# 0xPolygonZero/proof-protocol-decoder

Hardware: AMD Instinct MI355X
Metric: txn-proofs/sec (whole node), 256-txn synthetic block (higher is better)
Workload: dtype u64 (Goldilocks field)

## Files before the change

### include/bpg.h

```cpp
#ifndef BPG_H
#define BPG_H
#include <stddef.h>
#include <stdint.h>

#ifdef __cplusplus
extern "C" {
#endif

typedef enum {
  BP_OK = 0,
  BP_ERR_ABORTED = -1,
  BP_ERR_INVALID_INPUT = -2,
  BP_ERR_RANGE = -3,
  BP_ERR_DEVICE = -4,
  BP_ERR_VERIFY = -5,
  BP_ERR_UNSUPPORTED = -6
} bp_status;

const char* bp_last_error(void);
const char* bp_version(void);
int bp_device_count(void);
int bp_use_blocking_sync(int device);
int bp_host_wait_mode(int device);



#define BP_NTT_MAX_COLS 65535u

enum { BP_NTT_FWD_BR2NAT = 0, BP_NTT_INV_NAT2BR = 1, BP_NTT_FWD_NAT = 2, BP_NTT_INV_NAT = 3 };
int bp_ntt_batch(uint64_t* d_cols, uint32_t log_n, uint32_t n_cols, uint64_t col_stride, int dir,
                 void* stream);

int bp_intt_batch(const uint64_t* d_values, uint64_t in_stride, uint64_t* d_coeffs_out, uint64_t out_stride,
                  uint32_t log_n, uint32_t n_cols, void* stream);

int bp_lde_batch(const uint64_t* d_in, uint64_t in_stride, uint64_t* d_coeffs_out, uint64_t coeffs_stride,
                 uint64_t* d_lde_out, uint64_t lde_stride, uint32_t log_n, uint32_t rate_bits,
                 uint32_t n_cols, int from_coeffs, void* stream);

int bp_debug_copy_u64(const uint64_t* d_in, uint64_t* d_out, uint64_t n, void* stream);

int bp_debug_field_ops(const uint64_t* d_a, const uint64_t* d_b, uint64_t* d_out, uint64_t n, void* stream);
int bp_debug_mul_pow2(const uint64_t* d_a, uint64_t* d_out, uint64_t n, void* stream);

void bp_tune_quad_threshold(uint64_t n_perms);
void bp_tune_merkle_fused(int mode);
void bp_tune_merkle_wide(int log2_parents);
void bp_tune_poseidon_mx(int on);
void bp_tune_poseidon_mx_sets(int sets);
void bp_tune_poseidon_grouped(int on);
void bp_tune_assume_loaded(int mode);
void bp_tune_rec_batch(int n);
void bp_tune_side_lanes(int n);
void bp_tune_rec_riders(int on);
void bp_tune_txn_group(int n);
void bp_tune_rec_group(int mode);
int bp_debug_rec_batch_histogram(uint64_t* out, uint32_t n, int reset);
void bp_tune_witness_threads(int n);
void bp_tune_host_wait(int mode);
void bp_tune_host_poseidon(int mode);
int bp_debug_poseidon_host(uint64_t* states, size_t n);
void bp_tune_k5_spread(int on);
uint32_t bp_debug_poseidon_group_ops(uint32_t K);
int bp_debug_poseidon_group_tables(uint32_t K, uint32_t r0, uint8_t* out_ops, int32_t* out_cform, int32_t* out_cmain,
                                   int32_t* out_max_plane_sum);
// ... 326 lines not shown
```

### proof_protocol_decoder_amd/_abi.py

```python
import ctypes as C
from ctypes import POINTER as P

vp, cp, i, sz, dbl = C.c_void_p, C.c_char_p, C.c_int, C.c_size_t, C.c_double
u8, u32, u64, i32, i64 = C.c_uint8, C.c_uint32, C.c_uint64, C.c_int32, C.c_int64
u8p, u32p, u64p, i32p, szp = P(u8), P(u32), P(u64), P(i32), P(sz)
u8pp = P(u8p)

BP_OK, BP_ERR_ABORTED, BP_ERR_INVALID_INPUT, BP_ERR_RANGE, BP_ERR_DEVICE, BP_ERR_VERIFY, BP_ERR_UNSUPPORTED = 0, -1, -2, -3, -4, -5, -6
STATUS_NAMES = {v: k for k, v in list(globals().items()) if k == "BP_OK" or k.startswith("BP_ERR_")}
BP_SET_SKIP_LINK_CHECK = 1
BP_NUM_TABLES, BP_IR_WORDS, BP_PV_WORDS = 7, 25, 13

KNOBS = ("quad_threshold", "assume_loaded", "merkle_fused", "merkle_wide", "poseidon_mx", "poseidon_mx_sets",
         "poseidon_grouped", "ntt_mx", "ntt_split", "k5_spread", "host_wait", "host_poseidon", "rec_batch",
         "witness_threads", "side_lanes")


def _u32s(*names):
    return [(n, u32) for n in names]


class AirFamily(C.Structure):
    _fields_ = _u32s("first_index", "count", "kind", "degree")

# ... 96 lines not shown

class ShardOptions(C.Structure):
    _fields_ = _u32s("n_threads", "tree_shape")


ShardLeafFn = C.CFUNCTYPE(i, vp, u32, u8pp, szp)
ShardAggFn = C.CFUNCTYPE(i, vp, u8p, sz, i, u8p, sz, i, u8pp, szp)

_cfg, _conf, _wit, _opt, _gi = P(StarkCfg), P(BpConfig), P(TxnWitness), P(ShardOptions), P(GiOptions)
_trace = (i, [vp, u64, u32, vp, vp])
_check = [u32, _cfg, vp, u64, vp, u64p, u32, u64p, u32p, P(AirViolation), u32, u32p]
_knob, _ir_flag, _buf = (None, [i]), (i, [u64p, i]), [u8pp, szp]
PROTOTYPES = {
    "bp_last_error": (cp, []),
    "bp_version": (cp, []),
    "bp_device_count": (i, []),
    "bp_use_blocking_sync": (i, [i]),
    "bp_host_wait_mode": (i, [i]),
    "bp_ntt_batch": (i, [vp, u32, u32, u64, i, vp]),
    "bp_intt_batch": (i, [vp, u64, vp, u64, u32, u32, vp]),
    "bp_lde_batch": (i, [vp, u64, vp, u64, vp, u64, u32, u32, u32, i, vp]),
    "bp_debug_copy_u64": (i, [vp, vp, u64, vp]),
    "bp_debug_field_ops": (i, [vp, vp, vp, u64, vp]),
    "bp_debug_mul_pow2": (i, [vp, vp, u64, vp]),
    "bp_tune_quad_threshold": (None, [u64]),
    "bp_tune_merkle_fused": _knob,
    "bp_tune_merkle_wide": _knob,
    "bp_tune_poseidon_mx": _knob,
    "bp_tune_poseidon_mx_sets": _knob,
    "bp_tune_poseidon_grouped": _knob,
    "bp_tune_assume_loaded": _knob,
    "bp_tune_rec_batch": _knob,
    "bp_tune_side_lanes": _knob,
    "bp_tune_rec_riders": _knob,
    "bp_tune_txn_group": _knob,
    "bp_tune_rec_group": _knob,
    "bp_debug_rec_batch_histogram": (i, [u64p, u32, i]),
    "bp_tune_witness_threads": _knob,
    "bp_tune_host_wait": _knob,
    "bp_tune_host_poseidon": _knob,
    "bp_debug_poseidon_host": (i, [vp, sz]),
    "bp_tune_k5_spread": _knob,
    "bp_debug_poseidon_group_ops": (u32, [u32]),
    "bp_debug_poseidon_group_tables": (i, [u32, u32, u8p, i32p, i32p, i32p]),
    "bp_tune_ntt_split": _knob,
    "bp_tune_ntt_mx": _knob,
# ... 103 lines not shown
```

### proof_protocol_decoder_amd/csrc/air.hpp

```cpp
#pragma once
#include <cstdint>
#include <type_traits>
#include "gl.hpp"
#if defined(__HIP__)
#include "poseidon.cuh"
#endif

namespace bpg {
namespace air {

constexpr uint32_t SYNTHETIC = 0, KECCAK_F = 1, LOGIC = 2, MEMORY = 3, ARITHMETIC = 4, BYTE_PACKING = 5, KECCAK_SPONGE = 6, ARITHMETIC_MUL = 7, PLONK = 8, COUNT = 9;

struct Shape {
  uint32_t air_id, n_cols, n_const, deg_pow;
};

template <class T>
struct Ops;

#if defined(__HIP__)
template <>
struct Ops<uint64_t> {
  typedef uint64_t T;
  static __device__ __forceinline__ T k(uint64_t c) { return c; }
  static __device__ __forceinline__ T add(T a, T b) { return gl::addc(a, b); }
  static __device__ __forceinline__ T sub(T a, T b) { return gl::subc(a, b); }
  static __device__ __forceinline__ T mul(T a, T b) { return gl::mulc(a, b); }
  static __device__ __forceinline__ T dbl(T a) { return gl::addc(a, a); }
  static __device__ __forceinline__ void mul4(const T (&a)[4], const T (&b)[4], T (&r)[4]) {
    __builtin_amdgcn_sched_barrier(0);
    gl::mul_n<4>(a, b, r);
    gl::canon_n<4>(r);
    __builtin_amdgcn_sched_barrier(0);
  }
  static __device__ __forceinline__ void mul4_lazy(const T (&a)[4], const T (&b)[4], T (&r)[4]) {
    __builtin_amdgcn_sched_barrier(0);
    gl::mul_n<4>(a, b, r);
    __builtin_amdgcn_sched_barrier(0);
  }
  static __device__ __forceinline__ T add_lazy(T a_any, T b) { return gl::add(a_any, b); }
  static __device__ __forceinline__ T sub_lazy(T a_any, T b) { return gl::sub(a_any, b); }
  static __device__ __forceinline__ T mul7(T a_any) { return gl::mul7(a_any); }
};
#endif
template <>
struct Ops<gl::Ext> {
  typedef gl::Ext T;
  static T k(uint64_t c) { return gl::ext(c); }
  static T add(T a, T b) { return gl::add(a, b); }
  static T sub(T a, T b) { return gl::sub(a, b); }
  static T mul(T a, T b) { return gl::mul(a, b); }
  static T dbl(T a) { return gl::add(a, a); }
  static void mul4(const T (&a)[4], const T (&b)[4], T (&r)[4]) {
    for (int i = 0; i < 4; i++) r[i] = gl::mul(a[i], b[i]);
  }
  static void mul4_lazy(const T (&a)[4], const T (&b)[4], T (&r)[4]) { mul4(a, b, r); }
  static T add_lazy(T a, T b) { return gl::add(a, b); }
  static T sub_lazy(T a, T b) { return gl::sub(a, b); }
  static T mul7(T a) { return gl::scale(a, 7); }
};

GL_HD uint64_t poseidon_rc(uint32_t i) {
  constexpr uint64_t RC[360] = {
#include "poseidon_rc.inc"
  };
  return RC[i];
}
GL_HD uint32_t poseidon_mds_entry(uint32_t r, uint32_t c) {
  constexpr uint32_t C[12] = {17, 15, 41, 16, 2, 28, 13, 13, 39, 18, 34, 20};
  return C[(c + 12 - r) % 12] + ((r | c) == 0 ? 8u : 0u);
}
template <class T>
struct PoseidonOps {
  typedef Ops<T> F;
  static GL_HD T sbox(T x) {
    const T x2 = F::mul(x, x), x4 = F::mul(x2, x2), x3 = F::mul(x2, x);
    return F::mul(x3, x4);
  }
  static GL_HD void sbox_all(T (&s)[12]) {
    for (uint32_t i = 0; i < 12; i++) s[i] = sbox(s[i]);
  }
  static GL_HD void mds_rc(T (&s)[12], int next) {
    T o[12];
    for (uint32_t r = 0; r < 12; r++) {
      T acc = F::k(next >= 0 ? poseidon_rc(12 * (uint32_t)next + r) : 0);
      for (uint32_t c = 0; c < 12; c++) acc = F::add(acc, F::mul(F::k(poseidon_mds_entry(r, c)), s[c]));
      o[r] = acc;
    }
    for (uint32_t r = 0; r < 12; r++) s[r] = o[r];
  }
  static GL_HD void mds_rc_word0(T (&s)[12], int next) { mds_rc(s, next); }
  static GL_HD T add_rc0(T x, uint32_t i) { return F::add(x, F::k(poseidon_rc(i))); }
};
#if defined(__HIP__)
template <>
struct PoseidonOps<uint64_t> {
  static __device__ __forceinline__ uint64_t sbox(uint64_t x) { return gl::canon(poseidon::sbox(x)); }
  static __device__ __forceinline__ void sbox_all(uint64_t (&s)[12]) { poseidon::sbox_all(s); }
  static __device__ __forceinline__ void mds_rc(uint64_t (&s)[12], int next) {
    if (next >= 0) poseidon::mds<true>(s, poseidon::RC + 12 * next);
    else poseidon::mds<false>(s, nullptr);
#pragma unroll
    for (int i = 0; i < 12; i++) s[i] = gl::canon(s[i]);
  }
  static __device__ __forceinline__ void mds_rc_word0(uint64_t (&s)[12], int next) {
    poseidon::mds<true>(s, poseidon::RC + 12 * next);
    s[0] = gl::canon(s[0]);
  }
  static __device__ __forceinline__ uint64_t add_rc0(uint64_t x, uint32_t i) { return gl::addc(x, poseidon::RC[i]); }
};
#endif

namespace synthetic {
GL_HD uint32_t n_constraints(const Shape& s) { return 3 * (s.n_cols / 4); }
GL_HD uint32_t per_unit(const Shape& s) {
  const uint32_t G = s.n_cols / 4, u = (G + 47) / 48;
  return u < 8 ? 8 : u;
}
GL_HD uint32_t n_units(const Shape& s) {
  const uint32_t G = s.n_cols / 4, pu = per_unit(s);
  return (G + pu - 1) / pu;
}
template <class T, class Row, class Emit>
GL_HD void eval_unit(const Shape& s, uint32_t unit, const Row& row, Emit& out) {
  typedef Ops<T> F;
  const uint32_t G = s.n_cols / 4, pu = per_unit(s), g0 = unit * pu, g1 = g0 + pu < G ? g0 + pu : G;
#pragma unroll 1
  for (uint32_t g = g0; g < g1; g++) {
    const T a = row.loc(4 * g), b = row.loc(4 * g + 1), c = row.loc(4 * g + 2), d = row.loc(4 * g + 3);
    const T dn = row.nxt(4 * g + 3);
    const T q = s.n_const ? row.cst(g % s.n_const) : F::k(1);
    const T x4[4] = {a, q, a, a}, y4[4] = {b, a, b, b};
    T p4[4];
    F::mul4(x4, y4, p4);
    const T ab = p4[0], qa = p4[1];
    T t = F::mul(ab, c);
    if (s.deg_pow == 3) t = F::mul(F::mul(t, t), t);
    out.all(3 * g, F::sub(F::sub(c, ab), qa));
    out.transition(3 * g + 1, F::sub(F::sub(dn, t), b));
    out.first(3 * g + 2, F::sub(F::sub(d, a), b));
  }
}
}

namespace keccak {
constexpr uint32_t N_COLS = 2431, N_CONSTRAINTS = 2826, N_UNITS = 11;
constexpr uint32_t COL_STEP = 0, COL_A = 24, COL_C = 74, COL_CP = 394, COL_AP = 714, COL_APP = 2314, COL_APP0_BITS = 2364,
                   COL_APPP = 2428, COL_G = 2430;
constexpr uint32_t F0 = 0, F1 = 24, F2 = 48, F3 = 2032, F4 = 2352, F5 = 2672, F6 = 2722, F7 = 2772, F8 = 2774, F9 = 2776;
GL_HD uint64_t round_constant(uint32_t i) {
  constexpr uint64_t RC[24] = {
      0x0000000000000001ULL, 0x0000000000008082ULL, 0x800000000000808aULL, 0x8000000080008000ULL,
      0x000000000000808bULL, 0x0000000080000001ULL, 0x8000000080008081ULL, 0x8000000000008009ULL,
      0x000000000000008aULL, 0x0000000000000088ULL, 0x0000000080008009ULL, 0x000000008000000aULL,
      0x000000008000808bULL, 0x800000000000008bULL, 0x8000000000008089ULL, 0x8000000000008003ULL,
      0x8000000000008002ULL, 0x8000000000000080ULL, 0x000000000000800aULL, 0x800000008000000aULL,
      0x8000000080008081ULL, 0x8000000000008080ULL, 0x0000000080000001ULL, 0x8000000080008008ULL};
  return RC[i];
}
GL_HD uint32_t rho(uint32_t l) {
  constexpr uint8_t R[25] = {0, 1, 62, 28, 27, 36, 44, 6, 55, 20, 3, 10, 43, 25, 39, 41, 45, 15, 21, 8, 18, 2, 61, 56, 14};
  return R[l];
}
// ... 665 lines not shown
#pragma unroll
    for (uint32_t i = 0; i < 4; i++) {
      lhs[i] = row.loc(H_IN + i);
      rhs[i] = row.loc(H_IN + 4 + i);
      dl[i] = row.loc(H_DELTA + i);
      pr[i] = F::sub(rhs[i], lhs[i]);
    }
    const T s4[4] = {sw, sw, sw, sw};
    F::mul4(s4, pr, g);
#pragma unroll
    for (uint32_t i = 0; i < 4; i++) {
      const T d = F::sub(dl[i], g[i]);
      out.all(G5 + 1 + i, SELECTOR ? F::mul(qh, d) : d);
      st[i] = H::add_rc0(F::add(lhs[i], dl[i]), i);
      st[4 + i] = H::add_rc0(F::sub(rhs[i], dl[i]), 4 + i);
      st[8 + i] = H::add_rc0(row.loc(H_IN + 8 + i), 8 + i);
    }
    const T bit = F::mul(sw, F::sub(sw, F::k(1)));
    out.all(G5, SELECTOR ? F::mul(qh, bit) : bit);
  }
  auto check12 = [&](uint32_t col0, uint32_t idx0) {
#pragma unroll
    for (uint32_t i0 = 0; i0 < 12; i0 += 4) {
      T d[4], g[4];
#pragma unroll
      for (uint32_t i = 0; i < 4; i++) {
        const T wv = row.loc(col0 + i0 + i);
        d[i] = F::sub(wv, st[i0 + i]);
        st[i0 + i] = wv;
      }
      if (SELECTOR) F::mul4(q4, d, g);
#pragma unroll
      for (uint32_t i = 0; i < 4; i++) out.all(idx0 + i0 + i, SELECTOR ? g[i] : d[i]);
    }
  };
#pragma unroll 1
  for (uint32_t r = 1; r <= 3; r++) {
    H::sbox_all(st);
    H::mds_rc(st, (int)r);
    check12(H_FULL1 + 12 * (r - 1), G4 + 12 * (r - 1));
  }
  H::sbox_all(st);
  H::mds_rc_word0(st, 4);
#pragma unroll 1
  for (uint32_t r = 4; r <= 25; r++) {
    const T pv = row.loc(H_PART + r - 4);
    const T d = F::sub(pv, st[0]);
    out.all(G4 + 36 + (r - 4), SELECTOR ? F::mul(qh, d) : d);
    st[0] = H::sbox(pv);
    if (r < 25) H::mds_rc_word0(st, (int)r + 1);
    else H::mds_rc(st, (int)r + 1);
  }
#pragma unroll 1
// ... 3 lines not shown
    H::mds_rc(st, r < 29 ? (int)r + 1 : -1);
  }
  check12(H_OUT, G4 + 106);
}
template <class T, class Row, class Emit>
GL_HD void eval_chunk_unit(uint32_t u, uint32_t ctl_base, const uint64_t ctl[4], const Row& row, Emit& out) {
  typedef Ops<T> F;
  T w[8], sg[8];
#pragma unroll
  for (uint32_t i = 0; i < 8; i++) w[i] = row.loc(8 * u + i);
#pragma unroll
  for (uint32_t i = 0; i < 8; i++) sg[i] = row.cst(CST_SIGMA + 8 * u + i);
  const T qa = row.cst(CST_ARITH), qs = row.cst(CST_SBOX), c0 = row.cst(CST_C0), c1 = row.cst(CST_C1);
  const T x = row.x(), kp = F::k(chunk_shift(u));
  const T beta[2] = {F::k(ctl[0]), F::k(ctl[2])}, gamma[2] = {F::k(ctl[1]), F::k(ctl[3])};
  T bkx[2];
  {
    const T l1[4] = {w[0], w[4], c1, c1}, r1[4] = {w[1], w[5], w[2], w[6]};
    T p1[4];
    F::mul4(l1, r1, p1);
    const T l2[4] = {c0, c0, beta[0], beta[1]}, r2[4] = {p1[0], p1[1], x, x};
    T p2[4];
    F::mul4(l2, r2, p2);
    const T t0 = F::sub(F::add(p2[0], p1[2]), w[3]), t1 = F::sub(F::add(p2[1], p1[3]), w[7]);
    const T l3[4] = {qa, qa, p2[2], p2[3]}, r3[4] = {t0, t1, kp, kp};
    T p3[4];
    F::mul4(l3, r3, p3);
    out.all(G0 + 2 * u, p3[0]);
    out.all(G0 + 2 * u + 1, p3[1]);
    bkx[0] = p3[2];
    bkx[1] = p3[3];
  }
  T half[2][4];
#pragma unroll
  for (uint32_t c = 0; c < 2; c++) {
    const T b4[4] = {beta[c], beta[c], beta[c], beta[c]};
    T pn[4], pd[4];
#pragma unroll
    for (uint32_t h = 0; h < 2; h++) {
      const T s4[4] = {sg[4 * h], sg[4 * h + 1], sg[4 * h + 2], sg[4 * h + 3]};
      T bs[4], tn[4], td[4];
      F::mul4_lazy(b4, s4, bs);
#pragma unroll
      for (uint32_t i = 0; i < 4; i++) {
        const T wg = F::add(w[4 * h + i], gamma[c]);
        tn[i] = F::add_lazy(bkx[c], wg);
        td[i] = F::add_lazy(bs[i], wg);
        bkx[c] = F::mul7(bkx[c]);
      }
      const T l4[4] = {tn[0], tn[2], td[0], td[2]}, r4[4] = {tn[1], tn[3], td[1], td[3]};
      T q4[4];
      F::mul4_lazy(l4, r4, q4);
      pn[2 * h] = q4[0]; pn[2 * h + 1] = q4[1]; pd[2 * h] = q4[2]; pd[2 * h + 1] = q4[3];
    }
    const T l4[4] = {pn[0], pn[2], pd[0], pd[2]}, r4[4] = {pn[1], pn[3], pd[1], pd[3]};
    F::mul4_lazy(l4, r4, half[c]);
  }
  {
    const T l4[4] = {half[0][0], half[0][2], half[1][0], half[1][2]}, r4[4] = {half[0][1], half[0][3], half[1][1], half[1][3]};
    T nd[4];
    F::mul4_lazy(l4, r4, nd);
    const uint32_t k = u + 1;
    T cur[2], prev[2];
#pragma unroll
    for (uint32_t c = 0; c < 2; c++) {
      cur[c] = row.aux(10 * c + (k < 10 ? k : 0));
      prev[c] = k == 1 ? row.aux_nxt(10 * c) : row.aux(10 * c + k - 1);
    }
    const T m4[4] = {cur[0], prev[0], cur[1], prev[1]}, n4[4] = {nd[1], nd[0], nd[3], nd[2]};
    T g4[4];
    F::mul4(m4, n4, g4);
    out.all(ctl_base + u, F::sub(g4[0], g4[1]));
    out.all(ctl_base + 11 + u, F::sub(g4[2], g4[3]));
    if (u == 9) {
      out.first(ctl_base + 10, F::sub(cur[0], F::k(1)));
      out.first(ctl_base + 21, F::sub(cur[1], F::k(1)));
    }
  }
  if (u < 6) {
    const uint32_t n_here = u < 5 ? 2 : 1;
    const T qs4[4] = {qs, qs, qs, qs};
    T pend[4] = {F::k(0), F::k(0), F::k(0), F::k(0)};
#pragma unroll
    for (uint32_t e = 0; e < 2; e++) {
      if (e >= n_here) break;
      const uint32_t i = 2 * u + e, col = COL_SBOX + 5 * i;
      const T xs = row.loc(col), x2 = row.loc(col + 1), x4 = row.loc(col + 2), x6 = row.loc(col + 3), x7 = row.loc(col + 4);
      const T l4[4] = {xs, x2, x4, x6}, r4[4] = {xs, x2, x2, xs};
      T p4[4], d4[4], g4[4];
      F::mul4(l4, r4, p4);
      d4[0] = F::sub(x2, p4[0]); d4[1] = F::sub(x4, p4[1]); d4[2] = F::sub(x6, p4[2]); d4[3] = F::sub(x7, p4[3]);
      F::mul4(qs4, d4, g4);
#pragma unroll
      for (uint32_t q = 0; q < 4; q++) out.all(G1 + 4 * i + q, g4[q]);
      pend[2 * e] = F::sub(xs, w[4 * e]);
      pend[2 * e + 1] = F::sub(x7, w[4 * e + 3]);
    }
    T w4[4];
    F::mul4(qs4, pend, w4);
    out.all(G2 + 4 * u, w4[0]);
    out.all(G2 + 4 * u + 1, w4[1]);
    if (n_here == 2) {
      out.all(G2 + 4 * u + 2, w4[2]);
      out.all(G2 + 4 * u + 3, w4[3]);
    }
  }
  if (u == 0) {
#pragma unroll
    for (uint32_t j = 0; j < 4; j++) out.first(G3 + j, F::sub(w[j], F::k(row.pub(j))));
  }
}
template <class T, class Row, class Emit>
GL_HD void eval_unit(uint32_t u, uint32_t ctl_base, const uint64_t ctl[4], const Row& row, Emit& out) {
  if (u == 10) eval_hash_unit<T>(row, out);
// ... 306 lines not shown
```

### proof_protocol_decoder_amd/csrc/gl.hpp

```cpp
#pragma once
#include <cstdint>
#include <hip/hip_runtime.h>

#define GL_HD __host__ __device__ __forceinline__

namespace gl {

constexpr uint64_t P = 0xFFFFFFFF00000001ULL;
constexpr uint64_t EPS = 0xFFFFFFFFULL;
constexpr uint64_t GENERATOR = 7;
constexpr uint64_t TWO_ADIC_ROOT = 1753635133440165772ULL;
constexpr uint64_t W = 7;

#if defined(__HIP__)
namespace cc {
typedef uint64_t mask;
__device__ __forceinline__ uint64_t mad_co(uint32_t a, uint32_t b, uint64_t c, mask& co) {
  uint64_t d;
  asm("v_mad_u64_u32 %0, %1, %2, %3, %4" : "=v"(d), "=s"(co) : "v"(a), "v"(b), "v"(c));
  return d;
}
__device__ __forceinline__ uint64_t mad_eps_co(uint32_t a, uint64_t c, mask& co) {
  uint64_t d;
  asm("v_mad_u64_u32 %0, %1, %2, -1, %3" : "=v"(d), "=s"(co) : "v"(a), "v"(c));
// ... 20 lines not shown
  return d;
}
__device__ __forceinline__ uint32_t sub_co(uint32_t a, uint32_t b, mask& co) {
  uint32_t d;
  asm("v_sub_co_u32_e64 %0, %1, %2, %3" : "=v"(d), "=s"(co) : "v"(a), "v"(b));
  return d;
}
__device__ __forceinline__ uint32_t subb_co(uint32_t a, uint32_t b, mask ci, mask& co) {
  uint32_t d;
  asm("s_nop 1\n\tv_subb_co_u32_e64 %0, %1, %2, %3, %4" : "=v"(d), "=s"(co) : "v"(a), "v"(b), "s"(ci));
  return d;
}
__device__ __forceinline__ uint32_t subb0_co(uint32_t a, mask ci, mask& co) {
  uint32_t d;
  asm("s_nop 1\n\tv_subbrev_co_u32_e64 %0, %1, 0, %2, %3" : "=v"(d), "=s"(co) : "v"(a), "s"(ci));
  return d;
}
__device__ __forceinline__ uint32_t sel_eps(mask m) {
  uint32_t d;
  asm("s_nop 1\n\tv_cndmask_b32_e64 %0, 0, -1, %1" : "=v"(d) : "s"(m));
  return d;
}
__device__ __forceinline__ uint64_t mk64(uint32_t lo, uint32_t hi) { return ((uint64_t)hi << 32) | lo; }
#include "gl_cc.inc"
}
#endif
GL_HD uint64_t canon(uint64_t a) {
  return a >= P ? a - P : a;
}

GL_HD uint64_t add(uint64_t a, uint64_t b) {
  uint64_t s = a + b;
  return s < b ? s + EPS : s;
}
GL_HD uint64_t sub(uint64_t a, uint64_t b) {
  uint64_t d = a - b;
  return a < b ? d - EPS : d;
}
GL_HD uint64_t addc(uint64_t a, uint64_t b) {
  uint64_t s = a + b;
  return (s < a || s >= P) ? s - P : s;
}
GL_HD uint64_t subc(uint64_t a, uint64_t b) {
  return a >= b ? a - b : a + (P - b);
}
GL_HD uint64_t negc(uint64_t a) {
  return a ? P - a : 0;
}

GL_HD uint64_t reduce128(uint64_t lo, uint64_t hi) {
  uint64_t hh = hi >> 32, hl = hi & EPS;
  uint64_t t0 = lo - hh;
  if (lo < hh) t0 -= EPS;
  uint64_t t1 = (hl << 32) - hl;
  uint64_t r = t0 + t1;
  return r < t1 ? r + EPS : r;
}

GL_HD void mul_wide(uint64_t a, uint64_t b, uint64_t& lo, uint64_t& hi) {
#if defined(__HIP_DEVICE_COMPILE__)
  uint32_t a0 = (uint32_t)a, a1 = (uint32_t)(a >> 32), b0 = (uint32_t)b, b1 = (uint32_t)(b >> 32);
  uint64_t p00 = (uint64_t)a0 * b0;
  uint64_t mid = (uint64_t)a0 * b1 + (p00 >> 32);
  uint64_t mid2 = (uint64_t)a1 * b0 + (uint32_t)mid;
  hi = (uint64_t)a1 * b1 + (mid >> 32) + (mid2 >> 32);
  lo = (mid2 << 32) | (uint32_t)p00;
#else
  unsigned __int128 x = (unsigned __int128)a * b;
  lo = (uint64_t)x;
  hi = (uint64_t)(x >> 64);
// ... 98 lines not shown
  cc::subb_co_o(hi, b2, ah, bh, b1);
  cc::addc0_co(lo, b3, b2);
#pragma unroll
  for (int i = 0; i < N; i++) b2[i] &= ~b3[i];
  cc::subb0_cv(hi, b2);
#pragma unroll
  for (int i = 0; i < N; i++) r[i] = cc::mk64(lo[i], hi[i]);
}
template <int N>
__device__ __forceinline__ void canon_n(uint64_t (&a)[N]) {
  uint32_t lo[N], hi[N], tl[N], th[N];
  cc::mask k[N], c[N];
#pragma unroll
  for (int i = 0; i < N; i++) {
    lo[i] = (uint32_t)a[i]; hi[i] = (uint32_t)(a[i] >> 32);
  }
  cc::add_m1_co_o(tl, k, lo);
  cc::addc0_co_o(th, c, hi, k);
  cc::sel(lo, tl, c);
  cc::sel(hi, th, c);
#pragma unroll
  for (int i = 0; i < N; i++) a[i] = cc::mk64(lo[i], hi[i]);
}
#endif
GL_HD uint64_t mul_pow2_portable(uint64_t x, unsigned S) {
  if (S < 64) return reduce128(x << S, S ? x >> (64 - S) : 0);
  const unsigned s = S - 64;
  const uint64_t lo = x << s, hi = s ? x >> (64 - s) : 0;
  return sub(reduce128(0, lo), hi << 32);
}
#if defined(__HIP__)
__device__ __forceinline__ void shl96(uint64_t x, int s, uint32_t& l0, uint32_t& l1, uint32_t& l2) {
  const uint32_t x0 = (uint32_t)x, x1 = (uint32_t)(x >> 32);
  l0 = x0 << s;
  l1 = (x1 << s) | (x0 >> (32 - s));
  l2 = x1 >> (32 - s);
}
__device__ __forceinline__ uint64_t mul_pow2_lo(uint64_t x, int s) {
  uint32_t l0, l1, l2;
  shl96(x, s, l0, l1, l2);
  cc::mask c3, b3, cx;
  const uint64_t V = cc::mad_eps_co(l2, cc::mk64(l0, l1), c3);
  const uint32_t t0 = cc::subb0_co((uint32_t)V, c3, b3);
  const uint32_t t1 = cc::addc0_co((uint32_t)(V >> 32), c3 & ~b3, cx);
  return cc::mk64(t0, t1);
}
// ... 166 lines not shown
  const uint64_t e30 = mul(sq_n(e24, 6), e6);
  const uint64_t e31 = mul(sq_n(e30, 1), e1);
  const uint64_t hi = sq_n(e31, 1);
  const uint64_t lo = mul(hi, a);
  return mulc(sq_n(hi, 32), lo);
}
GL_HD uint64_t root(unsigned k) {
  uint64_t r = TWO_ADIC_ROOT;
  for (unsigned i = k; i < 32; i++) r = mulc(r, r);
  return r;
}

struct Ext {
  uint64_t c0, c1;
};
GL_HD Ext ext(uint64_t a, uint64_t b = 0) { return Ext{a, b}; }
GL_HD bool eq(Ext a, Ext b) { return a.c0 == b.c0 && a.c1 == b.c1; }
GL_HD Ext add(Ext a, Ext b) { return Ext{addc(a.c0, b.c0), addc(a.c1, b.c1)}; }
GL_HD Ext sub(Ext a, Ext b) { return Ext{subc(a.c0, b.c0), subc(a.c1, b.c1)}; }
GL_HD uint64_t mul7(uint64_t x) {
  const uint64_t p = (uint64_t)(uint32_t)x * 7u;
  const uint64_t m = (x >> 32) * 7u + (p >> 32);
  const uint64_t u = (m << 32) | (uint32_t)p;
  const uint64_t t = u + (m >> 32) * EPS;
  return t < u ? t + EPS : t;
}
GL_HD Ext mul(Ext a, Ext b) {
#if defined(__HIP_DEVICE_COMPILE__)
  const uint64_t x[4] = {a.c0, a.c1, a.c0, a.c1}, y[4] = {b.c0, b.c1, b.c1, b.c0};
  uint64_t r[4];
  mul_n<4>(x, y, r);
  return Ext{addc(canon(r[0]), canon(mul7(r[1]))), addc(canon(r[2]), canon(r[3]))};
#else
  uint64_t c0 = addc(mulc(a.c0, b.c0), mulc(W, mulc(a.c1, b.c1)));
  uint64_t c1 = addc(mulc(a.c0, b.c1), mulc(a.c1, b.c0));
  return Ext{c0, c1};
#endif
}
GL_HD Ext scale(Ext a, uint64_t s) { return Ext{mulc(a.c0, s), mulc(a.c1, s)}; }
GL_HD Ext pow(Ext a, uint64_t e) {
  Ext r = ext(1);
  while (e) {
    if (e & 1) r = mul(r, a);
    a = mul(a, a);
    e >>= 1;
  }
  return r;
}
GL_HD Ext inv(Ext a) {
  uint64_t n = subc(mulc(a.c0, a.c0), mulc(W, mulc(a.c1, a.c1)));
  uint64_t ni = inv(n);
  return Ext{mulc(a.c0, ni), mulc(negc(a.c1), ni)};
}

GL_HD uint32_t bitrev(uint32_t x, unsigned bits) {
// ... 11 lines not shown
```

### proof_protocol_decoder_amd/csrc/hash_kernels.hip

```cpp
#include <atomic>
#include <cstring>
#include <memory>
#include <mutex>
#include <vector>
#include "common.hpp"
#include "poseidon.cuh"
#include "poseidon_mx.cuh"
#include "stark_kernels.hpp"
#include "tune.hpp"

namespace {

__global__ void __launch_bounds__(256) perm_batch_kernel(uint64_t* __restrict__ states, uint64_t n) {
  uint64_t i = blockIdx.x * (uint64_t)blockDim.x + threadIdx.x;
  if (i >= n) return;
  uint64_t s[12];
#pragma unroll
  for (int k = 0; k < 12; k++) s[k] = states[i * 12 + k];
  poseidon::permute(s);
#pragma unroll
  for (int k = 0; k < 12; k++) states[i * 12 + k] = gl::canon(s[k]);
}

__global__ void __launch_bounds__(256) __attribute__((amdgpu_waves_per_eu(4, 8)))
// ... 482 lines not shown
    if (i >= n) break;
    const uint64_t cb = gl::canon(y[k]);
    out[0 * n + i] = gl::canon(gl::mul(x[k], y[k]));
    out[1 * n + i] = gl::canon(r4[k]);
    out[2 * n + i] = k ? gl::canon(r3[k - 1]) : gl::canon(r4[0]);
    uint64_t lo, hi;
    gl::mul_wide(x[k], y[k], lo, hi);
    out[3 * n + i] = gl::canon(gl::reduce128(lo, hi));
    out[4 * n + i] = gl::canon(gl::add(x[k], cb));
    out[5 * n + i] = gl::canon(gl::sub(x[k], cb));
    out[6 * n + i] = gl::dot_reduce(d[k]);
    out[7 * n + i] = gl::canon(gl::mul7(x[k]));
    out[8 * n + i] = gl::inv(gl::canon(x[k]));
    const gl::Ext e = gl::mul(gl::Ext{gl::canon(x[k]), cb}, gl::Ext{cb, gl::canon(x[k] ^ y[k])});
    out[9 * n + i] = e.c0;
    out[10 * n + i] = e.c1;
    out[11 * n + i] = gl::canon(sum4[k]);
    out[12 * n + i] = gl::canon(dif4[k]);
    out[13 * n + i] = cx4[k];
    out[14 * n + i] = cy[k];
  }
}

}

namespace bpg {

static std::atomic<int> g_active_provers{0};
void prover_active(int delta) { g_active_provers.fetch_add(delta, std::memory_order_relaxed); }
int provers_active() { return g_active_provers.load(std::memory_order_relaxed); }
bool device_loaded() {
  const int a = tune().assume_loaded.load(std::memory_order_relaxed);
  return a < 0 ? g_active_provers.load(std::memory_order_relaxed) >= 6 : a != 0;
}
bool poseidon_mx() { return tune().poseidon_mx.load(std::memory_order_relaxed) != 0; }
uint64_t quad_threshold() {
  const uint64_t t = tune().quad_threshold.load(std::memory_order_relaxed);
  if (t) return t;
  const bool loaded = device_loaded();
  if (poseidon_mx()) return (uint64_t)1 << (loaded ? 13 : 19);
  return (uint64_t)1 << (loaded ? 13 : 17);
}
int mx_sets(uint64_t n) {
  if (!poseidon_mx()) return 0;
  const int f = tune().poseidon_mx_sets.load(std::memory_order_relaxed);
  if (f) return f;
// ... 145 lines not shown
  BPG_LAUNCH_CHECK();
  return merkle_upper_levels(d_digests, log_leaves, cap_height, st, nullptr, nullptr);
}

}

extern "C" {

int bp_debug_copy_u64(const uint64_t* d_in, uint64_t* d_out, uint64_t n, void* stream) {
  if (!d_in || !d_out) return bpg::fail(BP_ERR_INVALID_INPUT, "bp_debug_copy_u64: null buffer");
  calib_copy_u64_kernel<<<4096, 256, 0, bpg::as_stream(stream)>>>(d_in, d_out, n);
  BPG_LAUNCH_CHECK();
  return BP_OK;
}

int bp_debug_field_ops(const uint64_t* d_a, const uint64_t* d_b, uint64_t* d_out, uint64_t n, void* stream) {
  if (!n) return BP_OK;
  if (!d_a || !d_b || !d_out) return bpg::fail(BP_ERR_INVALID_INPUT, "bp_debug_field_ops: null buffer");
  field_ops_kernel<<<bpg::ceil_div(bpg::ceil_div(n, 4), 256), 256, 0, bpg::as_stream(stream)>>>(d_a, d_b, d_out, n);
  BPG_LAUNCH_CHECK();
  return BP_OK;
}

int bp_debug_mul_pow2(const uint64_t* d_a, uint64_t* d_out, uint64_t n, void* stream) {
  if (!n) return BP_OK;
  if (!d_a || !d_out) return bpg::fail(BP_ERR_INVALID_INPUT, "bp_debug_mul_pow2: null buffer");
  mul_pow2_kernel<<<bpg::ceil_div(bpg::ceil_div(n, 4), 256), 256, 0, bpg::as_stream(stream)>>>(d_a, d_out, n);
  BPG_LAUNCH_CHECK();
  return BP_OK;
}

int bp_debug_poseidon_mx_cin(uint32_t* out) {
  if (!out) return bpg::fail(BP_ERR_INVALID_INPUT, "bp_debug_poseidon_mx_cin: null buffer");
  static const poseidon::mx::CinTable t = poseidon::mx::make_cin_table();
  for (int i = 0; i < poseidon::mx::CIN_WORDS; i++) out[i] = t.v[i];
  return BP_OK;
}

uint32_t bp_debug_poseidon_group_ops(uint32_t K) { return K >= 2 && K <= 8 ? (uint32_t)poseidon::group::layout((int)K).n_ops : 0; }
int bp_debug_poseidon_group_tables(uint32_t K, uint32_t r0, uint8_t* out_ops, int32_t* out_cform, int32_t* out_cmain,
                                   int32_t* out_max_plane_sum) try {
  if (!out_ops || !out_cform || !out_cmain) return bpg::fail(BP_ERR_INVALID_INPUT, "bp_debug_poseidon_group_tables: null output");
  poseidon::group::Tables t;
  if (!poseidon::group::build((int)K, (int)r0, &t))
    return bpg::fail(BP_ERR_INVALID_INPUT, "bp_debug_poseidon_group_tables: no such group (K=%u r0=%u)", K, r0);
  std::memcpy(out_ops, t.ops.data(), t.ops.size());
// ... 66 lines not shown
```

### proof_protocol_decoder_amd/csrc/ntt.hip

```cpp
#include <atomic>
#include <map>
#include <mutex>
#include <tuple>
#include <cstring>
#include <memory>
#include "common.hpp"
#include "gl.hpp"
#include "mx_arith.cuh"
#include "tune.hpp"

namespace {

constexpr uint32_t LOG_BLK_MAX = 14;

template <int LOGR, bool J0 = false>
__device__ __forceinline__ void dif_butterflies(uint64_t (&x)[1 << LOGR], const uint64_t* __restrict__ tw,
                                                uint32_t j, uint32_t log_sub, uint32_t tw_shift) {
  constexpr int R = 1 << LOGR, NB = R / 2;
#pragma unroll
  for (int s = 0; s < LOGR; s++) {
    const int half = R >> (s + 1);
    if constexpr (NB % 4 == 0) {
#pragma unroll
      for (int k0 = 0; k0 < NB; k0 += 4) {
// ... 300 lines not shown
}

template <int L>
__device__ __forceinline__ uint32_t swz(uint32_t i) {
  uint32_t x;
  if (L == 14) x = (((i >> 6) & 7u) << 2) ^ ((i >> 9) & 31u);
  else if (L == 13) x = (((i >> 5) & 15u) << 1) ^ ((i >> 9) & 15u);
  else x = (((i >> 8) & 1u) << 4) ^ ((i >> 7) & 1u) ^ (((i >> 9) & 7u) << 1);
  return i ^ x;
}
__device__ __forceinline__ uint32_t insert4(uint32_t t, uint32_t m, uint32_t b) {
  return ((t >> b) << (b + 4)) | (m << b) | (t & ((1u << b) - 1));
}
template <int R, int SH, bool CONTIG, bool DIF>
__device__ __forceinline__ void sub_butterflies(uint64_t (&x)[16], const uint64_t* __restrict__ tw, uint32_t j,
                                                uint32_t j_step_log, uint32_t log_sub, uint32_t tw_shift,
                                                const uint64_t* __restrict__ lay) {
  if constexpr (R == 4) {
    if (DIF) dif16<CONTIG>(x, lay, j, log_sub);
    else dit16<CONTIG>(x, lay, j, log_sub);
    return;
  }
  constexpr int G = 16 >> R;
#pragma unroll
  for (int g = 0; g < G; g++) {
    uint64_t y[1 << R];
#pragma unroll
    for (int u = 0; u < (1 << R); u++) y[u] = CONTIG ? x[(g << R) + u] : x[g + (u << SH)];
    const uint32_t jj = CONTIG ? 0u : j + ((uint32_t)g << j_step_log);
    if (DIF) dif_butterflies<R, CONTIG>(y, tw, jj, log_sub, tw_shift);
    else dit_butterflies<R, CONTIG>(y, tw, jj, log_sub, tw_shift);
#pragma unroll
    for (int u = 0; u < (1 << R); u++) {
      if (CONTIG) x[(g << R) + u] = y[u];
      else x[g + (u << SH)] = y[u];
    }
  }
}

struct Ntt16Args {
  const uint64_t* in;
  uint64_t in_stride;
  uint64_t* out;
  uint64_t out_stride, out_coset_stride;
  const uint64_t* tw;
  const uint64_t* scale;
// ... 741 lines not shown
```

### proof_protocol_decoder_amd/ops.py

```python
import contextlib
import ctypes as C

import numpy as np
import torch

from ._lib import KNOBS, StarkCfg, call_for_buffer, check, lib, own

NTT_FWD_BR2NAT, NTT_INV_NAT2BR, NTT_FWD_NAT, NTT_INV_NAT = 0, 1, 2, 3


def _stream():
    return torch.cuda.current_stream().cuda_stream


_tuned_active = False


@contextlib.contextmanager
def tuned(**knobs):
    global _tuned_active
    if _tuned_active:
        raise RuntimeError("ops.tuned() inside ops.tuned(): name all the knobs in one call")
    unknown = sorted(set(knobs) - set(KNOBS))
    if unknown:
# ... 39 lines not shown

def lde_batch(inp, rate_bits, from_coeffs=False):
    _require_cuda(inp)
    n_cols, n = inp.shape
    coeffs = torch.empty_like(inp)
    lde = torch.empty((n_cols, n << rate_bits), dtype=torch.int64, device=inp.device)
    check(own().bp_lde_batch(inp.data_ptr(), n, coeffs.data_ptr(), n, lde.data_ptr(), n << rate_bits,
                             n.bit_length() - 1, rate_bits, n_cols, int(from_coeffs), _stream()))
    return coeffs, lde


def poseidon_perm_batch_(states):
    _require_cuda(states)
    check(own().bp_poseidon_perm_batch(states.data_ptr(), states.numel() // 12, _stream()))
    return states


def field_ops(a, b):
    _require_cuda(a)
    _require_cuda(b)
    n = a.numel()
    out = torch.empty((15, n), dtype=torch.int64, device=a.device)
    check(own().bp_debug_field_ops(a.data_ptr(), b.data_ptr(), out.data_ptr(), n, _stream()))
    return out


def mul_pow2(a):
    _require_cuda(a)
    n = a.numel()
    out = torch.empty((21, n), dtype=torch.int64, device=a.device)
    check(own().bp_debug_mul_pow2(a.data_ptr(), out.data_ptr(), n, _stream()))
    return out


AIR_SYNTHETIC, AIR_KECCAK_F = 0, 1
KECCAK_COLS = 2431
LOGIC_COLS = 524
MEMORY_COLS = 45
ARITHMETIC_COLS = 309
BYTE_PACKING_COLS = 299
KECCAK_SPONGE_COLS = 2414
ARITHMETIC_MUL_COLS = 1217
AIR_TRACES = {1: ("keccak", KECCAK_COLS, lambda log_n: (((1 << log_n) + 23) // 24, 25)),
              2: ("logic", LOGIC_COLS, lambda log_n: (1 << log_n, 9)),
              3: ("memory", MEMORY_COLS, lambda log_n: (1 << log_n, 11)),
              4: ("arithmetic", ARITHMETIC_COLS, lambda log_n: (1 << log_n, 9)),
# ... 402 lines not shown
```

Baseline: 38.70.

## Use inline-asm Goldilocks add/sub/canon and 4-wide batched field ops in AIR and NTT

Replaces the scalar device versions of canon, add, sub, addc, subc, negc and mul7 with inline-asm sequences that apply the epsilon correction through a compare, cndmask and mad. Constraint evaluation, the Poseidon canonicalisation and Ext mul are regrouped into 4-wide batched add/sub/canon calls fenced by sched barriers. NTT sub-butterflies with small radix are restructured to process four butterflies at a time with vectorised canon/add/sub/mul. A debug field_forms kernel is added to check the new forms; the hand-written asm and sched barriers risk correctness subtleties and may constrain the compiler's scheduling.

```diff
diff --git a/include/bpg.h b/include/bpg.h
--- a/include/bpg.h
+++ b/include/bpg.h
@@ -41,6 +41,7 @@
 int bp_debug_copy_u64(const uint64_t* d_in, uint64_t* d_out, uint64_t n, void* stream);
 
 int bp_debug_field_ops(const uint64_t* d_a, const uint64_t* d_b, uint64_t* d_out, uint64_t n, void* stream);
+int bp_debug_field_forms(const uint64_t* d_a, const uint64_t* d_b, uint64_t* d_out, uint64_t n, void* stream);
 int bp_debug_mul_pow2(const uint64_t* d_a, uint64_t* d_out, uint64_t n, void* stream);
 
 void bp_tune_quad_threshold(uint64_t n_perms);
diff --git a/proof_protocol_decoder_amd/_abi.py b/proof_protocol_decoder_amd/_abi.py
--- a/proof_protocol_decoder_amd/_abi.py
+++ b/proof_protocol_decoder_amd/_abi.py
@@ -142,6 +142,7 @@
     "bp_lde_batch": (i, [vp, u64, vp, u64, vp, u64, u32, u32, u32, i, vp]),
     "bp_debug_copy_u64": (i, [vp, vp, u64, vp]),
     "bp_debug_field_ops": (i, [vp, vp, vp, u64, vp]),
+    "bp_debug_field_forms": (i, [vp, vp, vp, u64, vp]),
     "bp_debug_mul_pow2": (i, [vp, vp, u64, vp]),
     "bp_tune_quad_threshold": (None, [u64]),
     "bp_tune_merkle_fused": _knob,
diff --git a/proof_protocol_decoder_amd/csrc/air.hpp b/proof_protocol_decoder_amd/csrc/air.hpp
--- a/proof_protocol_decoder_amd/csrc/air.hpp
+++ b/proof_protocol_decoder_amd/csrc/air.hpp
@@ -36,6 +36,21 @@
   static __device__ __forceinline__ void mul4_lazy(const T (&a)[4], const T (&b)[4], T (&r)[4]) {
     __builtin_amdgcn_sched_barrier(0);
     gl::mul_n<4>(a, b, r);
+    __builtin_amdgcn_sched_barrier(0);
+  }
+  static __device__ __forceinline__ void add4(const T (&a)[4], const T (&b)[4], T (&r)[4]) {
+    __builtin_amdgcn_sched_barrier(0);
+    gl::addc_n<4>(a, b, r);
+    __builtin_amdgcn_sched_barrier(0);
+  }
+  static __device__ __forceinline__ void sub4(const T (&a)[4], const T (&b)[4], T (&r)[4]) {
+    __builtin_amdgcn_sched_barrier(0);
+    gl::subc_n<4>(a, b, r);
+    __builtin_amdgcn_sched_barrier(0);
+  }
+  static __device__ __forceinline__ void add4_lazy(const T (&a_any)[4], const T (&b)[4], T (&r)[4]) {
+    __builtin_amdgcn_sched_barrier(0);
+    gl::add_n<4>(a_any, b, r);
     __builtin_amdgcn_sched_barrier(0);
   }
   static __device__ __forceinline__ T add_lazy(T a_any, T b) { return gl::add(a_any, b); }
@@ -55,6 +70,13 @@
     for (int i = 0; i < 4; i++) r[i] = gl::mul(a[i], b[i]);
   }
   static void mul4_lazy(const T (&a)[4], const T (&b)[4], T (&r)[4]) { mul4(a, b, r); }
+  static void add4(const T (&a)[4], const T (&b)[4], T (&r)[4]) {
+    for (int i = 0; i < 4; i++) r[i] = gl::add(a[i], b[i]);
+  }
+  static void sub4(const T (&a)[4], const T (&b)[4], T (&r)[4]) {
+    for (int i = 0; i < 4; i++) r[i] = gl::sub(a[i], b[i]);
+  }
+  static void add4_lazy(const T (&a)[4], const T (&b)[4], T (&r)[4]) { add4(a, b, r); }
   static T add_lazy(T a, T b) { return gl::add(a, b); }
   static T sub_lazy(T a, T b) { return gl::sub(a, b); }
   static T mul7(T a) { return gl::scale(a, 7); }
@@ -101,7 +123,14 @@
     if (next >= 0) poseidon::mds<true>(s, poseidon::RC + 12 * next);
     else poseidon::mds<false>(s, nullptr);
 #pragma unroll
-    for (int i = 0; i < 12; i++) s[i] = gl::canon(s[i]);
+    for (int g = 0; g < 3; g++) {
+      uint64_t w[4] = {s[4 * g], s[4 * g + 1], s[4 * g + 2], s[4 * g + 3]};
+      __builtin_amdgcn_sched_barrier(0);
+      gl::canon_n<4>(w);
+      __builtin_amdgcn_sched_barrier(0);
+#pragma unroll
+      for (int i = 0; i < 4; i++) s[4 * g + i] = w[i];
+    }
   }
   static __device__ __forceinline__ void mds_rc_word0(uint64_t (&s)[12], int next) {
     poseidon::mds<true>(s, poseidon::RC + 12 * next);
@@ -136,9 +165,13 @@
     const T ab = p4[0], qa = p4[1];
     T t = F::mul(ab, c);
     if (s.deg_pow == 3) t = F::mul(F::mul(t, t), t);
-    out.all(3 * g, F::sub(F::sub(c, ab), qa));
-    out.transition(3 * g + 1, F::sub(F::sub(dn, t), b));
-    out.first(3 * g + 2, F::sub(F::sub(d, a), b));
+    const T m1[4] = {c, dn, d, c}, s1[4] = {ab, t, a, ab}, s2[4] = {qa, b, b, qa};
+    T e1[4], e2[4];
+    F::sub4(m1, s1, e1);
+    F::sub4(e1, s2, e2);
+    out.all(3 * g, e2[0]);
+    out.transition(3 * g + 1, e2[1]);
+    out.first(3 * g + 2, e2[2]);
   }
 }
 }
@@ -850,13 +883,14 @@
   auto check12 = [&](uint32_t col0, uint32_t idx0) {
 #pragma unroll
     for (uint32_t i0 = 0; i0 < 12; i0 += 4) {
-      T d[4], g[4];
+      T d[4], g[4], wv[4], sv[4];
 #pragma unroll
       for (uint32_t i = 0; i < 4; i++) {
-        const T wv = row.loc(col0 + i0 + i);
-        d[i] = F::sub(wv, st[i0 + i]);
-        st[i0 + i] = wv;
-      }
+        wv[i] = row.loc(col0 + i0 + i);
+        sv[i] = st[i0 + i];
+        st[i0 + i] = wv[i];
+      }
+      F::sub4(wv, sv, d);
       if (SELECTOR) F::mul4(q4, d, g);
 #pragma unroll
       for (uint32_t i = 0; i < 4; i++) out.all(idx0 + i0 + i, SELECTOR ? g[i] : d[i]);
@@ -906,7 +940,12 @@
     const T l2[4] = {c0, c0, beta[0], beta[1]}, r2[4] = {p1[0], p1[1], x, x};
     T p2[4];
     F::mul4(l2, r2, p2);
-    const T t0 = F::sub(F::add(p2[0], p1[2]), w[3]), t1 = F::sub(F::add(p2[1], p1[3]), w[7]);
+    const T sa[4] = {p2[0], p2[1], p2[0], p2[1]}, sb[4] = {p1[2], p1[3], p1[2], p1[3]};
+    T sm[4], df[4];
+    F::add4(sa, sb, sm);
+    const T dw[4] = {w[3], w[7], w[3], w[7]};
+    F::sub4(sm, dw, df);
+    const T t0 = df[0], t1 = df[1];
     const T l3[4] = {qa, qa, p2[2], p2[3]}, r3[4] = {t0, t1, kp, kp};
     T p3[4];
     F::mul4(l3, r3, p3);
@@ -925,13 +964,16 @@
       const T s4[4] = {sg[4 * h], sg[4 * h + 1], sg[4 * h + 2], sg[4 * h + 3]};
       T bs[4], tn[4], td[4];
       F::mul4_lazy(b4, s4, bs);
+      const T wh[4] = {w[4 * h], w[4 * h + 1], w[4 * h + 2], w[4 * h + 3]}, g4[4] = {gamma[c], gamma[c], gamma[c], gamma[c]};
+      T wg[4], bk[4];
+      F::add4(wh, g4, wg);
 #pragma unroll
       for (uint32_t i = 0; i < 4; i++) {
-        const T wg = F::add(w[4 * h + i], gamma[c]);
-        tn[i] = F::add_lazy(bkx[c], wg);
-        td[i] = F::add_lazy(bs[i], wg);
+        bk[i] = bkx[c];
         bkx[c] = F::mul7(bkx[c]);
       }
+      F::add4_lazy(bk, wg, tn);
+      F::add4_lazy(bs, wg, td);
       const T l4[4] = {tn[0], tn[2], td[0], td[2]}, r4[4] = {tn[1], tn[3], td[1], td[3]};
       T q4[4];
       F::mul4_lazy(l4, r4, q4);
@@ -973,7 +1015,8 @@
       const T l4[4] = {xs, x2, x4, x6}, r4[4] = {xs, x2, x2, xs};
       T p4[4], d4[4], g4[4];
       F::mul4(l4, r4, p4);
-      d4[0] = F::sub(x2, p4[0]); d4[1] = F::sub(x4, p4[1]); d4[2] = F::sub(x6, p4[2]); d4[3] = F::sub(x7, p4[3]);
+      const T h4[4] = {x2, x4, x6, x7};
+      F::sub4(h4, p4, d4);
       F::mul4(qs4, d4, g4);
 #pragma unroll
       for (uint32_t q = 0; q < 4; q++) out.all(G1 + 4 * i + q, g4[q]);
diff --git a/proof_protocol_decoder_amd/csrc/gl.hpp b/proof_protocol_decoder_amd/csrc/gl.hpp
--- a/proof_protocol_decoder_amd/csrc/gl.hpp
+++ b/proof_protocol_decoder_amd/csrc/gl.hpp
@@ -66,30 +66,87 @@
   return d;
 }
 __device__ __forceinline__ uint64_t mk64(uint32_t lo, uint32_t hi) { return ((uint64_t)hi << 32) | lo; }
+__device__ __forceinline__ void add_eps_if_lt(uint64_t& x, uint64_t a, uint64_t b) {
+  uint32_t e;
+  asm("v_cmp_lt_u64_e64 vcc, %2, %3\n\ts_nop 1\n\tv_cndmask_b32_e64 %1, 0, -1, vcc\n\tv_mad_u64_u32 %0, vcc, %1, 1, %0"
+      : "+v"(x), "=&v"(e) : "v"(a), "v"(b) : "vcc");
+}
+__device__ __forceinline__ void add_eps_if_ge_p(uint64_t& x) {
+  uint32_t e;
+  asm("v_cmp_gt_u64_e64 vcc, %0, %2\n\ts_nop 1\n\tv_cndmask_b32_e64 %1, 0, -1, vcc\n\tv_mad_u64_u32 %0, vcc, %1, 1, %0"
+      : "+v"(x), "=&v"(e) : "s"(0xFFFFFFFF00000000ULL) : "vcc");
+}
+__device__ __forceinline__ void add_eps_if_lt_or_ge_p(uint64_t& x, uint64_t a) {
+  uint32_t e;
+  mask m;
+  asm("v_cmp_lt_u64_e64 vcc, %0, %3\n\tv_cmp_gt_u64_e64 %2, %0, %4\n\ts_or_b64 vcc, vcc, %2\n\t"
+      "v_cndmask_b32_e64 %1, 0, -1, vcc\n\tv_mad_u64_u32 %0, vcc, %1, 1, %0"
+      : "+v"(x), "=&v"(e), "=&s"(m) : "v"(a), "s"(0xFFFFFFFF00000000ULL) : "vcc", "scc");
+}
+__device__ __forceinline__ void sub_eps_if_lt(uint64_t& x, uint64_t a, uint64_t b) {
+  uint32_t e;
+  asm("v_cmp_lt_u64_e64 vcc, %2, %3\n\ts_nop 1\n\tv_cndmask_b32_e64 %1, 0, -15, vcc\n\tv_mad_i64_i32 %0, vcc, %1, %4, %0"
+      : "+v"(x), "=&v"(e) : "v"(a), "v"(b), "s"(0x11111111u) : "vcc");
+}
+__device__ __forceinline__ void sub_eps_if_ne0(uint64_t& x, uint64_t a) {
+  uint32_t e;
+  asm("v_cmp_ne_u64_e64 vcc, 0, %2\n\ts_nop 1\n\tv_cndmask_b32_e64 %1, 0, -15, vcc\n\tv_mad_i64_i32 %0, vcc, %1, %3, %0"
+      : "+v"(x), "=&v"(e) : "v"(a), "s"(0x11111111u) : "vcc");
+}
 #include "gl_cc.inc"
 }
 #endif
 GL_HD uint64_t canon(uint64_t a) {
+#if defined(__HIP_DEVICE_COMPILE__)
+  cc::add_eps_if_ge_p(a);
+  return a;
+#else
   return a >= P ? a - P : a;
+#endif
 }
 
 GL_HD uint64_t add(uint64_t a, uint64_t b) {
   uint64_t s = a + b;
+#if defined(__HIP_DEVICE_COMPILE__)
+  cc::add_eps_if_lt(s, s, b);
+  return s;
+#else
   return s < b ? s + EPS : s;
+#endif
 }
 GL_HD uint64_t sub(uint64_t a, uint64_t b) {
   uint64_t d = a - b;
+#if defined(__HIP_DEVICE_COMPILE__)
+  cc::sub_eps_if_lt(d, a, b);
+  return d;
+#else
   return a < b ? d - EPS : d;
+#endif
 }
 GL_HD uint64_t addc(uint64_t a, uint64_t b) {
   uint64_t s = a + b;
+#if defined(__HIP_DEVICE_COMPILE__)
+  cc::add_eps_if_lt_or_ge_p(s, a);
+  return s;
+#else
   return (s < a || s >= P) ? s - P : s;
+#endif
 }
 GL_HD uint64_t subc(uint64_t a, uint64_t b) {
+#if defined(__HIP_DEVICE_COMPILE__)
+  return sub(a, b);
+#else
   return a >= b ? a - b : a + (P - b);
+#endif
 }
 GL_HD uint64_t negc(uint64_t a) {
+#if defined(__HIP_DEVICE_COMPILE__)
+  uint64_t d = 0 - a;
+  cc::sub_eps_if_ne0(d, a);
+  return d;
+#else
   return a ? P - a : 0;
+#endif
 }
 
 GL_HD uint64_t reduce128(uint64_t lo, uint64_t hi) {
@@ -234,6 +291,29 @@
 #pragma unroll
   for (int i = 0; i < N; i++) a[i] = cc::mk64(lo[i], hi[i]);
 }
+template <int N>
+__device__ __forceinline__ void addc_n(const uint64_t (&a)[N], const uint64_t (&b)[N], uint64_t (&r)[N]) {
+  uint32_t al[N], ah[N], bl[N], bh[N], lo[N], hi[N], tl[N], th[N];
+  cc::mask c1[N], c2[N], k[N], c[N];
+#pragma unroll
+  for (int i = 0; i < N; i++) {
+    al[i] = (uint32_t)a[i]; ah[i] = (uint32_t)(a[i] >> 32); bl[i] = (uint32_t)b[i]; bh[i] = (uint32_t)(b[i] >> 32);
+  }
+  cc::add_co_o(lo, c1, al, bl);
+  cc::addc_co_o(hi, c2, ah, bh, c1);
+  cc::add_m1_co_o(tl, k, lo);
+  cc::addc0_co_o(th, c, hi, k);
+#pragma unroll
+  for (int i = 0; i < N; i++) c[i] |= c2[i];
+  cc::sel(lo, tl, c);
+  cc::sel(hi, th, c);
+#pragma unroll
+  for (int i = 0; i < N; i++) r[i] = cc::mk64(lo[i], hi[i]);
+}
+template <int N>
+__device__ __forceinline__ void subc_n(const uint64_t (&a)[N], const uint64_t (&b)[N], uint64_t (&r)[N]) {
+  sub_n<N>(a, b, r);
+}
 #endif
 GL_HD uint64_t mul_pow2_portable(uint64_t x, unsigned S) {
   if (S < 64) return reduce128(x << S, S ? x >> (64 - S) : 0);
@@ -446,15 +526,22 @@
   const uint64_t p = (uint64_t)(uint32_t)x * 7u;
   const uint64_t m = (x >> 32) * 7u + (p >> 32);
   const uint64_t u = (m << 32) | (uint32_t)p;
-  const uint64_t t = u + (m >> 32) * EPS;
+  uint64_t t = u + (m >> 32) * EPS;
+#if defined(__HIP_DEVICE_COMPILE__)
+  cc::add_eps_if_lt(t, t, u);
+  return t;
+#else
   return t < u ? t + EPS : t;
+#endif
 }
 GL_HD Ext mul(Ext a, Ext b) {
 #if defined(__HIP_DEVICE_COMPILE__)
   const uint64_t x[4] = {a.c0, a.c1, a.c0, a.c1}, y[4] = {b.c0, b.c1, b.c1, b.c0};
   uint64_t r[4];
   mul_n<4>(x, y, r);
-  return Ext{addc(canon(r[0]), canon(mul7(r[1]))), addc(canon(r[2]), canon(r[3]))};
+  r[1] = mul7(r[1]);
+  canon_n<4>(r);
+  return Ext{addc(r[0], r[1]), addc(r[2], r[3])};
 #else
   uint64_t c0 = addc(mulc(a.c0, b.c0), mulc(W, mulc(a.c1, b.c1)));
   uint64_t c1 = addc(mulc(a.c0, b.c1), mulc(a.c1, b.c0));
diff --git a/proof_protocol_decoder_amd/csrc/hash_kernels.hip b/proof_protocol_decoder_amd/csrc/hash_kernels.hip
--- a/proof_protocol_decoder_amd/csrc/hash_kernels.hip
+++ b/proof_protocol_decoder_amd/csrc/hash_kernels.hip
@@ -528,6 +528,45 @@
   }
 }
 
+__global__ void __launch_bounds__(256) field_forms_kernel(const uint64_t* __restrict__ a, const uint64_t* __restrict__ b,
+                                                          uint64_t* __restrict__ out, uint64_t n) {
+  const uint64_t i0 = (blockIdx.x * (uint64_t)blockDim.x + threadIdx.x) * 4;
+  if (i0 >= n) return;
+  uint64_t x[4], cx[4], cy[4], sum4[4], dif4[4];
+#pragma unroll
+  for (int k = 0; k < 4; k++) {
+    const uint64_t i = i0 + k < n ? i0 + k : n - 1;
+    x[k] = a[i];
+    cx[k] = gl::canon(x[k]);
+    cy[k] = gl::canon(b[i]);
+  }
+  __builtin_amdgcn_sched_barrier(0);
+  gl::addc_n<4>(cx, cy, sum4);
+  __builtin_amdgcn_sched_barrier(0);
+  gl::subc_n<4>(cx, cy, dif4);
+  __builtin_amdgcn_sched_barrier(0);
+#pragma unroll
+  for (int k = 0; k < 4; k++) {
+    const uint64_t i = i0 + k;
+    if (i >= n) break;
+    out[0 * n + i] = cx[k];
+    out[1 * n + i] = gl::add(x[k], cy[k]);
+    out[2 * n + i] = gl::sub(x[k], cy[k]);
+    out[3 * n + i] = gl::addc(cx[k], cy[k]);
+    out[4 * n + i] = gl::subc(cx[k], cy[k]);
+    out[5 * n + i] = gl::negc(cx[k]);
+    out[6 * n + i] = sum4[k];
+    out[7 * n + i] = dif4[k];
+    const gl::Ext e = gl::Ext{cx[k], cy[k]}, f = gl::Ext{cy[k], gl::canon(x[k] ^ b[i])};
+    const gl::Ext es = gl::add(e, f), ed = gl::sub(e, f);
+    out[8 * n + i] = es.c0;
+    out[9 * n + i] = es.c1;
+    out[10 * n + i] = ed.c0;
+    out[11 * n + i] = ed.c1;
+    out[12 * n + i] = gl::mul7(x[k]);
+  }
+}
+
 }
 
 namespace bpg {
@@ -719,6 +758,14 @@
   return BP_OK;
 }
 
+int bp_debug_field_forms(const uint64_t* d_a, const uint64_t* d_b, uint64_t* d_out, uint64_t n, void* stream) {
+  if (!n) return BP_OK;
+  if (!d_a || !d_b || !d_out) return bpg::fail(BP_ERR_INVALID_INPUT, "bp_debug_field_forms: null buffer");
+  field_forms_kernel<<<bpg::ceil_div(bpg::ceil_div(n, 4), 256), 256, 0, bpg::as_stream(stream)>>>(d_a, d_b, d_out, n);
+  BPG_LAUNCH_CHECK();
+  return BP_OK;
+}
+
 int bp_debug_mul_pow2(const uint64_t* d_a, uint64_t* d_out, uint64_t n, void* stream) {
   if (!n) return BP_OK;
   if (!d_a || !d_out) return bpg::fail(BP_ERR_INVALID_INPUT, "bp_debug_mul_pow2: null buffer");
diff --git a/proof_protocol_decoder_amd/csrc/ntt.hip b/proof_protocol_decoder_amd/csrc/ntt.hip
--- a/proof_protocol_decoder_amd/csrc/ntt.hip
+++ b/proof_protocol_decoder_amd/csrc/ntt.hip
@@ -346,6 +346,50 @@
     return;
   }
   constexpr int G = 16 >> R;
+  if constexpr (R < 3) {
+#pragma unroll
+    for (int s = 0; s < R; s++) {
+      const int dist = DIF ? (1 << R) >> (s + 1) : 1 << s;
+#pragma unroll
+      for (int e0 = 0; e0 < 8; e0 += 4) {
+        const int k = e0 / G, m = (k / dist) * 2 * dist + (k % dist);
+        const bool unit = CONTIG && (m & (dist - 1)) == 0;
+        int ia[4], ib[4];
+        uint64_t a[4], b[4], w[4], hi[4], lo[4];
+#pragma unroll
+        for (int i = 0; i < 4; i++) {
+          const int g = (e0 + i) % G;
+          ia[i] = CONTIG ? (g << R) + m : g + (m << SH);
+          ib[i] = CONTIG ? (g << R) + m + dist : g + ((m + dist) << SH);
+          a[i] = x[ia[i]];
+          b[i] = x[ib[i]];
+          if (!unit) {
+            const uint32_t jj = CONTIG ? 0u : j + ((uint32_t)g << j_step_log);
+            const uint32_t p = jj + ((uint32_t)(m & (dist - 1)) << log_sub);
+            w[i] = tw[p << (tw_shift + (DIF ? s : R - 1 - s))];
+          }
+        }
+        if constexpr (DIF) {
+          gl::canon_n<4>(b);
+          gl::add_n<4>(a, b, hi);
+          gl::sub_n<4>(a, b, lo);
+          if (!unit) gl::mul_n<4>(lo, w, lo);
+        } else {
+          if (!unit) gl::mul_n<4>(b, w, b);
+          gl::canon_n<4>(b);
+          gl::add_n<4>(a, b, hi);
+          gl::sub_n<4>(a, b, lo);
+        }
+#pragma unroll
+        for (int i = 0; i < 4; i++) {
+          x[ia[i]] = hi[i];
+          x[ib[i]] = lo[i];
+        }
+        __builtin_amdgcn_sched_barrier(0);
+      }
+    }
+    return;
+  }
 #pragma unroll
   for (int g = 0; g < G; g++) {
     uint64_t y[1 << R];
diff --git a/proof_protocol_decoder_amd/ops.py b/proof_protocol_decoder_amd/ops.py
--- a/proof_protocol_decoder_amd/ops.py
+++ b/proof_protocol_decoder_amd/ops.py
@@ -85,6 +85,15 @@
     n = a.numel()
     out = torch.empty((15, n), dtype=torch.int64, device=a.device)
     check(own().bp_debug_field_ops(a.data_ptr(), b.data_ptr(), out.data_ptr(), n, _stream()))
+    return out
+
+
+def field_forms(a, b):
+    _require_cuda(a)
+    _require_cuda(b)
+    n = a.numel()
+    out = torch.empty((13, n), dtype=torch.int64, device=a.device)
+    check(own().bp_debug_field_forms(a.data_ptr(), b.data_ptr(), out.data_ptr(), n, _stream()))
     return out
 
 
```

Result: no change. 38.80, median of 6 (+0.3%).
